# NVlabs/WarpConvNet

Hardware: AMD Instinct MI355X
Metric: M active voxels/sec fwd+bwd, SparseConv3d 64→128 k=3, 1/2/4/8 MI355X (higher is better)
Workload: dtype bf16; 1 GPU; configs[1]: one 1000000-voxel uniform (U) scene per GPU, SparseConv3d 64->128 k=3, bf16 autocast, kernel-map build + AB fwd + ABt dgrad + AtB wgrad per step; voxels_per_gpu=1000000, coord_order=generator, parallelism=dp1 (scene-sharded, grad all-reduce)

## Files before the change

warpconvnet_amd/csrc/kmap.hip:

```cpp
#include "kmap_cells.h"

namespace wcn {

constexpr int kBlockRows = 256;
constexpr int kThreads = 256;

__global__ void hash_prepare_kernel(uint4* __restrict__ slots, int64_t capacity) {
  const int64_t i = (int64_t)blockIdx.x * blockDim.x + threadIdx.x;
  if (i < capacity) slots[i] = make_uint4(0u, 0u, 0xFFFFFFFFu, 0u);
}

__global__ void hash_insert_kernel(Slot* __restrict__ slots, uint32_t capacity_mask, const int4* __restrict__ coords,
                                   int64_t n, int32_t* __restrict__ status) {
  const int64_t i = (int64_t)blockIdx.x * blockDim.x + threadIdx.x;
  if (i >= n) return;
  const int4 c = coords[i];
  if (!coord_in_range(c.x, c.y, c.z, c.w)) {
    atomicOr(status, (int)WCN_FLAG_COORD_RANGE);
    return;
  }
  const uint64_t key = pack_key(c.x, c.y, c.z, c.w);
  uint32_t s = hash_slot(key, capacity_mask);
  for (uint32_t attempts = 0; attempts <= capacity_mask; ++attempts) {
    unsigned long long* kp = reinterpret_cast<unsigned long long*>(&slots[s].key);
    const unsigned long long prev = atomicCAS(kp, 0ull, (unsigned long long)key);
    if (prev == 0ull || prev == key) {
      atomicMin(reinterpret_cast<unsigned int*>(&slots[s].value), (unsigned int)i);
      if (prev == key) atomicOr(status, (int)WCN_FLAG_DUPLICATE_COORD);
      return;
    }
    s = (s + 1) & capacity_mask;
  }
  atomicOr(status, (int)WCN_FLAG_TABLE_FULL);
}

__global__ void hash_search_kernel(const Slot* __restrict__ slots, uint32_t capacity_mask,
                                   const int4* __restrict__ queries, int64_t m, int32_t* __restrict__ results) {
  const int64_t i = (int64_t)blockIdx.x * blockDim.x + threadIdx.x;
  if (i >= m) return;
  const int4 q = queries[i];
  results[i] = slot_lookup(slots, capacity_mask, pack_key(q.x, q.y, q.z, q.w));
}

struct HashLookup {
  const Slot* slots;
  uint32_t cmask;
  __device__ __forceinline__ int operator()(int b, int x, int y, int z) const {
    return slot_lookup(slots, cmask, pack_key(b, x, y, z));
  }
};

struct CellLookup {
  const BSlot* slots;
  uint32_t cmask;
  CellTable t;
  __device__ __forceinline__ int operator()(int b, int x, int y, int z) const {
    const int xx = (x << (32 - kCoordBits)) >> (32 - kCoordBits);
    const int yy = (y << (32 - kCoordBits)) >> (32 - kCoordBits);
    const int zz = (z << (32 - kCoordBits)) >> (32 - kCoordBits);
    const int id = block_id_of(slots, cmask, make_int4(b, xx, yy, zz));
    int found = -1;
    if (id >= 0)
      found = t.cells[(int64_t)id * kCells + (((xx & (kBlk - 1)) * kBlk + (yy & (kBlk - 1))) * kBlk + (zz & (kBlk - 1)))];
    return found;
  }
};

template <int LPR, typename Lookup>
__global__ __launch_bounds__(kThreads) void kmap_probe_kernel(Lookup lookup, const int4* __restrict__ query, int64_t m,
                                                              KernelGeom g, int K, int kp, int mw, int32_t* __restrict__ nbr,
                                                              uint32_t* __restrict__ mask) {
  const int tid = threadIdx.x;
  constexpr int kRowsPerIter = 64 / LPR;
  const int lane = tid & 63;
  const int wave = tid >> 6;
  const int sub = lane % LPR;
  const int rsel = lane / LPR;
  const int64_t wave_row0 = (int64_t)blockIdx.x * kBlockRows + wave * 64;
  const int num_chunks = (kp + LPR - 1) / LPR;

  for (int kc = 0; kc < num_chunks; ++kc) {
    const int k = kc * LPR + sub;
    const bool k_real = k < K;
    const bool k_store = k < kp;
    const int l = k % g.kz;
    const int j = (k / g.kz) % g.ky;
    const int i = k / (g.kz * g.ky);
    const int ox = (i - g.cx) * g.dx, oy = (j - g.cy) * g.dy, oz = (l - g.cz) * g.dz;
#pragma unroll 4
    for (int it = 0; it < 64 / kRowsPerIter; ++it) {
      const int64_t row = wave_row0 + it * kRowsPerIter + rsel;
      int found = -1;
      if (row < m && k_real) {
        const int4 q = query[row];
        found = lookup(q.x, q.y * g.sx + ox, q.z * g.sy + oy, q.w * g.sz + oz);
      }
      if (row < m && k_store) nbr[row * kp + k] = found;
      const unsigned long long ball = __ballot(found >= 0);
      if (row < m && sub == 0) {
        const unsigned long long bits = (LPR == 64) ? ball : ((ball >> (rsel * LPR)) & ((1ull << (LPR & 63)) - 1ull));
        const int w0 = (kc * LPR) >> 5;
        if (w0 < mw) mask[row * mw + w0] = (uint32_t)bits;
        if (LPR == 64 && w0 + 1 < mw) mask[row * mw + w0 + 1] = (uint32_t)(bits >> 32);
      }
    }
  }
}

template <typename Lookup>
static int launch_probe(const Lookup& lookup, const void* table, const int32_t* query, int64_t m, const int32_t ksize[3],
                        const int32_t stride[3], const int32_t dilation[3], int32_t* nbr, uint32_t* mask, hipStream_t s) {
  if (m < 0 || !ksize || !stride || !dilation) return WCN_ERROR_INVALID_PARAMETERS;
  for (int d = 0; d < 3; ++d)
    if (ksize[d] < 1 || stride[d] < 1 || dilation[d] < 1) return WCN_ERROR_INVALID_PARAMETERS;
  const int64_t K64 = (int64_t)ksize[0] * ksize[1] * ksize[2];
  if (!valid_k(K64)) return WCN_ERROR_PROBLEM_NOT_SUPPORTED;
  if (m == 0) return WCN_SUCCESS;
  if (!table || !query || !nbr || !mask) return WCN_ERROR_INVALID_PARAMETERS;
  const int K = (int)K64, kp = wcn_kmap_row_pitch(K), mw = wcn_kmap_mask_words(K);
  const KernelGeom g = make_kernel_geom(ksize, stride, dilation);
  const dim3 grid((unsigned)ceil_div(m, kBlockRows)), block(kThreads);
#define WCN_PROBE(L) \
  hipLaunchKernelGGL((kmap_probe_kernel<L, Lookup>), grid, block, 0, s, lookup, (const int4*)query, m, g, K, kp, mw, nbr, mask)
  switch (lanes_per_row(kp)) {
    case 8: WCN_PROBE(8); break;
    case 16: WCN_PROBE(16); break;
    case 32: WCN_PROBE(32); break;
    default: WCN_PROBE(64); break;
  }
#undef WCN_PROBE
  return launch_status();
}

__global__ __launch_bounds__(256) void batch_indexed_coords_kernel(const int32_t* __restrict__ coords, int64_t n, int d,
                                                                   const int32_t* __restrict__ offsets, int num_batches,
                                                                   int32_t* __restrict__ out) {
  const int64_t i = (int64_t)blockIdx.x * blockDim.x + threadIdx.x;
  if (i >= n) return;
  const int b = last_offset_not_above(offsets, num_batches, i);
  if (d == 3) {
    const int32_t* c = coords + i * 3;
    *reinterpret_cast<int4*>(out + i * 4) = make_int4(b, c[0], c[1], c[2]);
  } else {
    out[i * (d + 1)] = b;
    for (int j = 0; j < d; ++j) out[i * (d + 1) + 1 + j] = coords[i * d + j];
  }
}

__device__ __forceinline__ uint64_t spread3(uint64_t v) {
  v &= 0x1FFFFFull;
  v = (v | (v << 32)) & 0x001F00000000FFFFull;
  v = (v | (v << 16)) & 0x001F0000FF0000FFull;
  v = (v | (v << 8)) & 0x100F00F00F00F00Full;
  v = (v | (v << 4)) & 0x10C30C30C30C30C3ull;
  v = (v | (v << 2)) & 0x1249249249249249ull;
  return v;
}

__global__ __launch_bounds__(256) void morton_code_kernel(const int32_t* __restrict__ coords, int64_t n, int d,
                                                          const int32_t* __restrict__ origin, int a0, int a1, int a2,
                                                          int64_t* __restrict__ codes) {
  const int64_t i = (int64_t)blockIdx.x * blockDim.x + threadIdx.x;
  if (i >= n) return;
  const int32_t* c = coords + i * d;
  const int sp = d - 3;
  int64_t v[3];
  const int ax[3] = {a0, a1, a2};
#pragma unroll
  for (int j = 0; j < 3; ++j) v[j] = (int64_t)c[sp + ax[j]] - (origin ? (int64_t)origin[sp + ax[j]] : 0);
  uint64_t m = spread3((uint64_t)v[0]) | (spread3((uint64_t)v[1]) << 1) | (spread3((uint64_t)v[2]) << 2);
  if (d == 4) {
    const int64_t b = (int64_t)c[0] - (origin ? (int64_t)origin[0] : 0);
    m = (m & 0x0000FFFFFFFFFFFFull) | ((uint64_t)b << 48);
  }
  codes[i] = (int64_t)m;
}

__global__ __launch_bounds__(kThreads) void kmap_transpose_kernel(const int32_t* __restrict__ nbr, int64_t m, int K,
                                                                  int kp, int tr, int32_t* __restrict__ pair_table) {
  extern __shared__ int s_tile[];
  const int64_t row0 = (int64_t)blockIdx.x * tr;
  const int pitch = kp + 1;
  for (int e = threadIdx.x; e < tr * kp; e += kThreads) {
    const int r = e / kp, k = e % kp;
    s_tile[r * pitch + k] = (row0 + r < m) ? nbr[(row0 + r) * kp + k] : -1;
  }
  __syncthreads();
  for (int e = threadIdx.x; e < tr * K; e += kThreads) {
    const int k = e / tr, r = e % tr;
    if (row0 + r < m) pair_table[(int64_t)k * m + row0 + r] = s_tile[r * pitch + k];
  }
}

__global__ void fill_i32_kernel(int32_t* __restrict__ p, int64_t n, int32_t v) {
  const int64_t i = (int64_t)blockIdx.x * blockDim.x + threadIdx.x;
  if (i < n) p[i] = v;
}

__global__ void kmap_pairs_to_table_kernel(const int32_t* __restrict__ in_maps, const int32_t* __restrict__ out_maps,
                                           const int32_t* __restrict__ offsets, int K, int kp, int mw, int64_t max_pairs,
                                           int by_in, int32_t* __restrict__ tbl, uint32_t* __restrict__ mask) {
  const int64_t p = (int64_t)blockIdx.x * blockDim.x + threadIdx.x;
  if (p >= max_pairs || p >= offsets[K]) return;
  const int k = last_offset_not_above(offsets, K, p);
  const int i = in_maps[p], o = out_maps[p];
  const int64_t row = by_in ? i : o;
  tbl[row * kp + k] = by_in ? o : i;
  atomicOr(&mask[row * mw + (k >> 5)], 1u << (k & 31));
}

}

using namespace wcn;

extern "C" {

int wcn_abi_version(void) { return 18; }

const char* wcn_status_string(int status) {
  switch (status) {
    case WCN_SUCCESS: return "Success";
    case WCN_ERROR_PROBLEM_NOT_SUPPORTED: return "Problem size not supported";
    case WCN_ERROR_KERNEL_INITIALIZATION: return "Kernel initialization failed";
    case WCN_ERROR_KERNEL_EXECUTION: return "Kernel execution failed";
    case WCN_ERROR_UNSUPPORTED_CONFIG: return "Unsupported precision/configuration";
    case WCN_ERROR_INVALID_PARAMETERS: return "Invalid parameters";
    case WCN_ERROR_MIXED_INPUT_UNSUPPORTED: return "Mixed input precision unsupported";
    default: return "Unknown error";
  }
}

static inline bool is_pow2(int64_t v) { return v > 0 && (v & (v - 1)) == 0; }

int wcn_hash_prepare(void* slots, int64_t capacity, wcn_stream_t stream) {
  if (!slots || !is_pow2(capacity) || capacity > (1ll << 31)) return WCN_ERROR_INVALID_PARAMETERS;
  hipLaunchKernelGGL(hash_prepare_kernel, dim3((unsigned)ceil_div(capacity, 256)), dim3(256), 0, (hipStream_t)stream,
                     (uint4*)slots, capacity);
  return launch_status();
}

int wcn_hash_insert(void* slots, int64_t capacity, const int32_t* coords, int64_t n, int32_t* status,
                    wcn_stream_t stream) {
  if (!slots || !is_pow2(capacity) || capacity > (1ll << 31) || n < 0 || !status) return WCN_ERROR_INVALID_PARAMETERS;
  if (n == 0) return WCN_SUCCESS;
  if (!coords) return WCN_ERROR_INVALID_PARAMETERS;
  hipLaunchKernelGGL(hash_insert_kernel, dim3((unsigned)ceil_div(n, 256)), dim3(256), 0, (hipStream_t)stream,
                     (Slot*)slots, (uint32_t)(capacity - 1), (const int4*)coords, n, status);
  return launch_status();
}

int wcn_hash_search(const void* slots, int64_t capacity, const int32_t* queries, int64_t m, int32_t* results,
                    wcn_stream_t stream) {
  if (!slots || !is_pow2(capacity) || m < 0) return WCN_ERROR_INVALID_PARAMETERS;
  if (m == 0) return WCN_SUCCESS;
  if (!queries || !results) return WCN_ERROR_INVALID_PARAMETERS;
  hipLaunchKernelGGL(hash_search_kernel, dim3((unsigned)ceil_div(m, 256)), dim3(256), 0, (hipStream_t)stream,
                     (const Slot*)slots, (uint32_t)(capacity - 1), (const int4*)queries, m, results);
  return launch_status();
}

int32_t wcn_kmap_row_pitch(int32_t num_offsets) { return (num_offsets + 7) & ~7; }
int32_t wcn_kmap_mask_words(int32_t num_offsets) { return (num_offsets + 31) / 32; }
int wcn_kmap_probe(const void* slots, int64_t capacity, const int32_t* query, int64_t m, const int32_t ksize[3],
                   const int32_t stride[3], const int32_t dilation[3], int32_t* nbr, uint32_t* mask,
                   wcn_stream_t stream) {
  if (!slots || !is_pow2(capacity)) return WCN_ERROR_INVALID_PARAMETERS;
  return launch_probe(HashLookup{(const Slot*)slots, (uint32_t)(capacity - 1)}, slots, query, m, ksize, stride, dilation, nbr,
                      mask, (hipStream_t)stream);
}

int wcn_kmap_probe_cells(const void* cells_workspace, int64_t n_in, int64_t max_blocks, const int32_t* query, int64_t m,
                         const int32_t ksize[3], const int32_t stride[3], const int32_t dilation[3], int32_t* nbr,
                         uint32_t* mask, wcn_stream_t stream) {
  if (n_in < 0 || max_blocks < 1) return WCN_ERROR_INVALID_PARAMETERS;
  const CellTable t = carve_cells(const_cast<void*>(cells_workspace), n_in, max_blocks);
  return launch_probe(CellLookup{t.slots, (uint32_t)(t.capacity - 1), t}, cells_workspace, query, m, ksize, stride, dilation,
                      nbr, mask, (hipStream_t)stream);
}

int wcn_batch_indexed_coords(const int32_t* coords, int64_t n, int32_t num_dims, const int32_t* offsets,
                             int32_t num_batches, int32_t* out, wcn_stream_t stream) {
  if (n < 0 || num_dims < 1 || num_dims > 8 || num_batches < 1) return WCN_ERROR_INVALID_PARAMETERS;
  if (n == 0) return WCN_SUCCESS;
  if (!coords || !out || (num_batches > 1 && !offsets)) return WCN_ERROR_INVALID_PARAMETERS;
  hipLaunchKernelGGL(batch_indexed_coords_kernel, dim3((unsigned)ceil_div(n, 256)), dim3(256), 0, (hipStream_t)stream, coords,
                     n, (int)num_dims, offsets, (int)num_batches, out);
  return launch_status();
}

int wcn_morton_code(const int32_t* coords, int64_t n, int32_t num_dims, const int32_t* origin, const int32_t axis[3],
                    int64_t* codes, wcn_stream_t stream) {
  if (n < 0 || (num_dims != 3 && num_dims != 4) || !axis) return WCN_ERROR_INVALID_PARAMETERS;
  int seen = 0;
  for (int j = 0; j < 3; ++j) {
    if (axis[j] < 0 || axis[j] > 2) return WCN_ERROR_INVALID_PARAMETERS;
    seen |= 1 << axis[j];
  }
  if (seen != 7) return WCN_ERROR_INVALID_PARAMETERS;
  if (n == 0) return WCN_SUCCESS;
  if (!coords || !codes) return WCN_ERROR_INVALID_PARAMETERS;
  hipLaunchKernelGGL(morton_code_kernel, dim3((unsigned)ceil_div(n, 256)), dim3(256), 0, (hipStream_t)stream, coords, n,
                     (int)num_dims, origin, (int)axis[0], (int)axis[1], (int)axis[2], codes);
  return launch_status();
}

int wcn_kmap_transpose(const int32_t* nbr, int64_t m, int32_t num_offsets, int32_t* pair_table, wcn_stream_t stream) {
  if (m < 0 || !valid_k(num_offsets)) return WCN_ERROR_INVALID_PARAMETERS;
  if (m == 0) return WCN_SUCCESS;
  if (!nbr || !pair_table) return WCN_ERROR_INVALID_PARAMETERS;
  const int kp = wcn_kmap_row_pitch(num_offsets);
  int tr = 64;
  while (tr > 1 && (size_t)tr * (kp + 1) * sizeof(int) > 64 * 1024) tr >>= 1;
  hipLaunchKernelGGL(kmap_transpose_kernel, dim3((unsigned)ceil_div(m, tr)), dim3(kThreads),
                     (size_t)tr * (kp + 1) * sizeof(int), (hipStream_t)stream, nbr, m, (int)num_offsets, kp, tr, pair_table);
  return launch_status();
}

static int pairs_to_table(const int32_t* in_maps, const int32_t* out_maps, const int32_t* offsets, int32_t K,
                          int64_t max_pairs, int64_t rows, int by_in, int32_t* tbl, uint32_t* mask, hipStream_t s) {
  if (!valid_k(K) || rows < 0 || max_pairs < 0 || !offsets) return WCN_ERROR_INVALID_PARAMETERS;
  if (rows == 0) return WCN_SUCCESS;
  if (!tbl || !mask) return WCN_ERROR_INVALID_PARAMETERS;
  const int kp = wcn_kmap_row_pitch(K), mw = wcn_kmap_mask_words(K);
  hipLaunchKernelGGL(fill_i32_kernel, dim3((unsigned)ceil_div(rows * kp, 256)), dim3(256), 0, s, tbl, rows * kp, -1);
  hipLaunchKernelGGL(fill_i32_kernel, dim3((unsigned)ceil_div(rows * mw, 256)), dim3(256), 0, s, (int32_t*)mask,
                     rows * mw, 0);
  if (max_pairs > 0) {
    if (!in_maps || !out_maps) return WCN_ERROR_INVALID_PARAMETERS;
    hipLaunchKernelGGL(kmap_pairs_to_table_kernel, dim3((unsigned)ceil_div(max_pairs, 256)), dim3(256), 0, s, in_maps,
                       out_maps, offsets, (int)K, kp, mw, max_pairs, by_in, tbl, mask);
  }
  return launch_status();
}

int wcn_kmap_reverse(const int32_t* in_maps, const int32_t* out_maps, const int32_t* offsets, int32_t num_offsets,
                     int64_t max_pairs, int64_t n_in, int32_t* rev_nbr, uint32_t* rev_mask, wcn_stream_t stream) {
  return pairs_to_table(in_maps, out_maps, offsets, num_offsets, max_pairs, n_in, 1, rev_nbr, rev_mask,
                        (hipStream_t)stream);
}

int wcn_kmap_from_csr(const int32_t* in_maps, const int32_t* out_maps, const int32_t* offsets, int32_t num_offsets,
                      int64_t max_pairs, int64_t n_out, int32_t* nbr, uint32_t* mask, wcn_stream_t stream) {
  return pairs_to_table(in_maps, out_maps, offsets, num_offsets, max_pairs, n_out, 0, nbr, mask, (hipStream_t)stream);
}

}
```

warpconvnet_amd/csrc/kmap_binned.hip:

```cpp
#include "kmap_cells.h"

namespace wcn {

constexpr int kInsertSample = 8;
constexpr int kInsertThreads = 512;
constexpr int kRowBufPitch = 66;
constexpr int kRowBufInts = (kCompactPitch + 1) * kRowBufPitch;
#ifndef WCN_NB_WPE
#define WCN_NB_WPE 3
#endif
constexpr int kNbWavesPerSimd = WCN_NB_WPE;
constexpr int kNbThreads = 256;

__device__ __forceinline__ int wrap_blk(int v) {
  const int bits = kBlkCoordBits;
  v &= (1 << bits) - 1;
  return (v ^ (1 << (bits - 1))) - (1 << (bits - 1));
}

__global__ void cell_prepare_kernel(uint4* __restrict__ slots, int64_t capacity, int32_t* __restrict__ ctr,
                                    uint32_t* __restrict__ halo, CellGeom g, int32_t* __restrict__ status) {
  const int64_t i = (int64_t)blockIdx.x * blockDim.x + threadIdx.x;
  if (i < capacity) slots[i] = make_uint4(0u, 0u, 0xFFFFFFFFu, 0u);
  if (i < 64) ctr[i] = 0;
  if (i == 0) *status = 0;
  if (i < g.halo_cells) {
    const int h3[3] = {g.hx, g.hy, g.hz};
    int t = (int)i, dir = 0;
    int sx = 0, sy = 0, sz = 0;
    for (; dir < 27; ++dir) {
      if (dir == 13) continue;
      const int dd[3] = {dir / 9 - 1, (dir / 3) % 3 - 1, dir % 3 - 1};
      sx = dd[0] ? h3[0] : kBlk; sy = dd[1] ? h3[1] : kBlk; sz = dd[2] ? h3[2] : kBlk;
      const int cells = sx * sy * sz;
      if (t < cells) break;
      t -= cells;
    }
    const int ddx = dir / 9 - 1, ddy = (dir / 3) % 3 - 1, ddz = dir % 3 - 1;
    const int tz = t % sz, ty = (t / sz) % sy, tx = t / (sz * sy);
    const int lx = ddx < 0 ? kBlk - g.hx + tx : tx;
    const int ly = ddy < 0 ? kBlk - g.hy + ty : ty;
    const int lz = ddz < 0 ? kBlk - g.hz + tz : tz;
    const int X = lx + kBlk * ddx + g.hx, Y = ly + kBlk * ddy + g.hy, Z = lz + kBlk * ddz + g.hz;
    halo[i] = ((uint32_t)dir << 27) | ((uint32_t)cell_index(lx, ly, lz) << 16) | (uint32_t)(X * g.px + Y * g.py + Z);
  }
}

__device__ __forceinline__ void store_cell(int32_t* cell, int row, bool strict) {
  if (strict) __hip_atomic_fetch_min(reinterpret_cast<uint32_t*>(cell), (uint32_t)row, __ATOMIC_RELAXED, __HIP_MEMORY_SCOPE_AGENT);
  else *cell = row;
}

template <int PHASE>
__global__ __launch_bounds__(kInsertThreads) void cell_insert_kernel(BSlot* __restrict__ slots, uint32_t cmask,
                                                          const int4* __restrict__ coords, int64_t n, CellTable t,
                                                          int32_t* __restrict__ status, int kp, int mw,
                                                          int32_t* __restrict__ nbr, uint32_t* __restrict__ mask,
                                                          int strict) {
  const bool compact = kp < 0;
  kp &= 0x7FFFFFFF;
  const int64_t tid = (int64_t)blockIdx.x * blockDim.x + threadIdx.x;
  const int64_t i = PHASE == 0 ? tid * kInsertSample : tid;
  const int lane = threadIdx.x & 63;
  bool live = i < n;
  int4 c = make_int4(0, 0, 0, 0);
  if (live) {
    c = coords[i];
    if (!coord_in_range(c.x, c.y, c.z, c.w)) {
      live = false;
      if (PHASE == 1) {
        atomicOr(status, (int)WCN_FLAG_COORD_RANGE);
        for (int k = 0; k < kp; ++k) nbr[i * kp + k] = compact ? 0 : -1;
        for (int w = 0; w < mw; ++w) mask[i * mw + w] = 0u;
      }
    }
  }
  int found = -1;
  int id = -1;
  bool created = false;
  uint64_t key = 0;
  if (live) {
    key = pack_key(c.x, c.y >> kBlkShift, c.z >> kBlkShift, c.w >> kBlkShift);
    uint32_t s = hash_slot(key, cmask);
    int idv = -1;
    for (uint32_t a = 0; a <= cmask; ++a) {
      unsigned long long* kptr = reinterpret_cast<unsigned long long*>(&slots[s].key);
      const uint4 v = *reinterpret_cast<const uint4*>(slots + s);
      unsigned long long cur = ((unsigned long long)v.y << 32) | v.x;
      if (cur == key) { found = (int)s; idv = (int)v.z; break; }
      if (cur == 0ull) {
        if (PHASE == 1) cur = __hip_atomic_load(kptr, __ATOMIC_RELAXED, __HIP_MEMORY_SCOPE_AGENT);
        if (cur == 0ull) {
          cur = atomicCAS(kptr, 0ull, (unsigned long long)key);
          if (cur == 0ull) {
            created = true;
            found = (int)s;
            break;
          }
        }
        if (cur == key) { found = (int)s; break; }
      }
      s = (s + 1) & cmask;
    }
    if (found < 0) atomicOr(status, (int)WCN_FLAG_TABLE_FULL);
    if (PHASE == 1 && idv >= 0 && !(idv & kIdLateBit)) id = idv;
  }
  __shared__ int s_made[kInsertThreads / 64 + 1];
  const int wave = threadIdx.x >> 6;
  const unsigned long long makers = __ballot(created);
  if (PHASE == 0) {
    if (lane == 0) s_made[wave] = __popcll(makers);
    __syncthreads();
    if (threadIdx.x == 0) {
      int tot = 0;
      for (int w = 0; w < kInsertThreads / 64; ++w) {
        const int c = s_made[w];
        s_made[w] = tot;
        tot += c;
      }
      s_made[kInsertThreads / 64] = tot > 0 ? atomicAdd(&t.ctr[0], tot) : 0;
    }
    __syncthreads();
  }
  if (makers != 0ull) {
    int base;
    if (PHASE == 0) {
      base = s_made[kInsertThreads / 64] + s_made[wave];
    } else {
      const int leader = __ffsll((long long)makers) - 1;
      base = 0;
      if (lane == leader) base = atomicAdd(&t.ctr[0], __popcll(makers));
      base = __shfl(base, leader);
    }
    int my_id = base + __popcll(makers & ((1ull << lane) - 1ull));
    if (!created) my_id = -1;
    if (my_id >= t.max_blocks) {
      atomicOr(status, (int)WCN_FLAG_TABLE_FULL);
      my_id = -1;
    }
    if (my_id >= 0) {
      t.blk_key[my_id] = key;
      slots[found].id = my_id | (PHASE == 1 ? kIdLateBit : 0);
    }
    unsigned long long todo = makers;
    while (todo != 0ull) {
      const int src = __ffsll((long long)todo) - 1;
      todo &= todo - 1ull;
      const int bid = __shfl(my_id, src);
      if (bid >= 0) {
        int4* gcells = reinterpret_cast<int4*>(t.cells + (int64_t)bid * kCells);
        gcells[lane] = make_int4(-1, -1, -1, -1);
        gcells[lane + 64] = make_int4(-1, -1, -1, -1);
      }
    }
  }
  if (PHASE == 0) return;
  if (live) mask[i * mw + (mw - 1)] = (id >= 0 || found < 0) ? kMaskUnwritten : kMaskDeferred;
  if (id >= 0) store_cell(t.cells + (int64_t)id * kCells + cell_of(c), (int)i, strict != 0);
}

__global__ __launch_bounds__(256) void cell_finish_kernel(const BSlot* __restrict__ slots, uint32_t cmask,
                                                          const int4* __restrict__ coords, int64_t n, CellTable t,
                                                          CellGeom g, int mw, const uint32_t* __restrict__ mask,
                                                          int strict) {
  const int64_t tid = (int64_t)blockIdx.x * blockDim.x + threadIdx.x;
  const int64_t nthreads = (int64_t)gridDim.x * blockDim.x;
  for (int64_t i = tid; i < n; i += nthreads) {
    if (mask[i * mw + (mw - 1)] != kMaskDeferred) continue;
    const int4 c = coords[i];
    const int id = block_id_of(slots, cmask, c);
    if (id < 0) continue;
    store_cell(t.cells + (int64_t)id * kCells + cell_of(c), (int)i, strict != 0);
  }
  const int lane = threadIdx.x & 63;
  int nblocks = t.ctr[0];
  if (nblocks > t.max_blocks) nblocks = (int)t.max_blocks;
  for (int64_t seq = tid >> 6; seq < nblocks; seq += nthreads >> 6) {
    const int id = (int)seq;
    int nid = -1;
    if (lane < 27) {
      const int ddx = lane / 9 - 1, ddy = (lane / 3) % 3 - 1, ddz = lane % 3 - 1;
      const bool needed = (ddx == 0 || g.hx > 0) && (ddy == 0 || g.hy > 0) && (ddz == 0 || g.hz > 0);
      if (lane == 13) nid = id;
      else if (needed) {
        const uint64_t key = t.blk_key[id];
        const int b = (int)((key >> 54) & kBatchMask);
        const int bx = wrap_blk((int)((key >> 36) & kCoordMask));
        const int by = wrap_blk((int)((key >> 18) & kCoordMask));
        const int bz = wrap_blk((int)(key & kCoordMask));
        const int s = block_find(slots, cmask, pack_key(b, wrap_blk(bx + ddx), wrap_blk(by + ddy), wrap_blk(bz + ddz)));
        if (s >= 0) {
          nid = slots[s].id;
          if (nid >= 0) nid &= ~kIdLateBit;
        }
      }
    }
    if (lane < 32) t.nbtab[(int64_t)id * 32 + lane] = nid;
  }
}

#ifdef WCN_PROF
__device__ unsigned long long g_bprof[4096 * 12];
#define BSTAMP(i) do { const unsigned long long now_ = wall_clock64(); prof_acc[i] += now_ - prof_prev; prof_prev = now_; } while (0)
#else
#define BSTAMP(i)
#endif

template <int LPR, bool FAST, bool COMPACT>
__global__ __launch_bounds__(kNbThreads) __attribute__((amdgpu_waves_per_eu(kNbWavesPerSimd))) void cell_neighbors_kernel(CellTable t, const uint32_t* __restrict__ halo,
                                                                    CellGeom g, int K, int kp, int mw,
                                                                    int32_t* __restrict__ nbr,
                                                                    uint32_t* __restrict__ mask,
                                                                    int32_t* __restrict__ status) {
  extern __shared__ int s_mem[];
  const int lane = threadIdx.x & 63, wave = threadIdx.x >> 6;
  uint32_t* s_halo = reinterpret_cast<uint32_t*>(s_mem);
  const int rounds = (g.halo_cells + 63) >> 6;
  const bool halo_regs = COMPACT && rounds <= 8;
  const int halo_pad = halo_regs ? 0 : rounds * 64;
  const int per_wave = g.cells + 4 + kCells / 2 + 8 + (COMPACT ? kRowBufInts : 0);
  int* s_grid = s_mem + halo_pad + wave * per_wave;
  unsigned short* s_own = reinterpret_cast<unsigned short*>(s_grid + g.cells + 4);
  const int null_cell = g.cells;
  for (int h = threadIdx.x; h < halo_pad; h += blockDim.x) s_halo[h] = h < g.halo_cells ? halo[h] : 0xFFFFFFFFu;
  if (lane == 0) s_grid[null_cell] = -1;
  __syncthreads();

  int nblocks = t.ctr[0];
  if (nblocks > t.max_blocks) nblocks = (int)t.max_blocks;
  const int gwave = blockIdx.x * (blockDim.x / 64) + wave;
  const int nwaves = gridDim.x * (blockDim.x / 64);
  constexpr int kVoxPerIter = 64 / LPR;
  const int sub = lane % LPR, vsel = lane / LPR;
  const int num_chunks = (kp + LPR - 1) / LPR;
  uint32_t he[8];
#pragma unroll
  for (int u = 0; u < 8; ++u) {
    const int idx = u * 64 + lane;
    uint32_t e = COMPACT && idx < g.halo_cells ? halo[idx] : 0xFFFFFFFFu;
    if (e == 0xFFFFFFFFu) e = (31u << 27) | (uint32_t)(g.cells + 1);
    he[u] = e;
  }
  auto load_head = [&](int seq, int& nb, int4& v0, int4& v1) {
    nb = -1;
    v0 = make_int4(-1, -1, -1, -1);
    v1 = v0;
    if (seq < nblocks) {
      if (lane < 27) nb = t.nbtab[(int64_t)seq * 32 + lane];
      const int4* own = reinterpret_cast<const int4*>(t.cells + (int64_t)seq * kCells) + lane * 2;
      v0 = own[0];
      v1 = own[1];
    }
  };
  int seq = gwave;
  int nb_c, nb_n;
  int4 c0, c1, n0, n1;
  load_head(seq, nb_c, c0, c1);
  load_head(seq + nwaves, nb_n, n0, n1);
  int hv[8];
  auto gather = [&](int nb, int r0) {
#pragma unroll
    for (int u = 0; u < 8; ++u) {
      hv[u] = -1;
      if (r0 + u < rounds) {
        const uint32_t e = s_halo[(r0 + u) * 64 + lane];
        const int nid = __shfl(nb, (int)((e >> 27) & 31u));
        if (e != 0xFFFFFFFFu && nid >= 0) hv[u] = t.cells[(int64_t)nid * kCells + ((e >> 16) & (kCells - 1))];
      }
    }
  };
  int nidv[8];
  auto gather8 = [&](int nb) {
#pragma unroll
    for (int u = 0; u < 8; ++u) nidv[u] = __shfl(nb, (int)(he[u] >> 27));
#pragma unroll
    for (int u = 0; u < 8; ++u)
      if (u < rounds) {
        const int safe = nidv[u] < 0 ? 0 : nidv[u];
        hv[u] = t.cells[(int64_t)safe * kCells + ((he[u] >> 16) & (kCells - 1))];
      }
  };
  auto scatter8 = [&]() {
#pragma unroll
    for (int u = 0; u < 8; ++u)
      if (u < rounds) s_grid[he[u] & 0xFFFFu] = nidv[u] >= 0 ? hv[u] : -1;
  };
  auto scatter_halo = [&](int r0) {
#pragma unroll
    for (int u = 0; u < 8; ++u)
      if (r0 + u < rounds) {
        const uint32_t e = s_halo[(r0 + u) * 64 + lane];
        if (e != 0xFFFFFFFFu) s_grid[e & 0xFFFFu] = hv[u];
      }
  };
  int* s_rows = s_grid + g.cells + 4 + kCells / 2 + 8;
  int pend_row = -1;
  auto flush_rows = [&](int row) {
    __builtin_amdgcn_fence(__ATOMIC_RELEASE, "wavefront");
    __builtin_amdgcn_wave_barrier();
    if (row >= 0) mask[row] = (uint32_t)s_rows[lane];
    const int piece = lane & 3;
    int rid[4];
    int4 v[4];
#pragma unroll
    for (int q = 0; q < 4; ++q) rid[q] = __shfl(row, (lane >> 2) + 16 * q);
#pragma unroll
    for (int q = 0; q < 4; ++q) {
      const int r = (lane >> 2) + 16 * q;
      v[q].x = s_rows[(piece * 4 + 0) * kRowBufPitch + r];
      v[q].y = s_rows[(piece * 4 + 1) * kRowBufPitch + r];
      v[q].z = s_rows[(piece * 4 + 2) * kRowBufPitch + r];
      v[q].w = s_rows[(piece * 4 + 3) * kRowBufPitch + r];
    }
#pragma unroll
    for (int q = 0; q < 4; ++q)
      if (rid[q] >= 0 && __popc((uint32_t)s_rows[(lane >> 2) + 16 * q]) >= 4 * piece) {
        if (FAST)
          *reinterpret_cast<int4*>(reinterpret_cast<char*>(nbr) + (__umul24((uint32_t)rid[q], kCompactPitch * 4u) + (uint32_t)piece * 16u)) = v[q];
        else
          *reinterpret_cast<int4*>(nbr + (int64_t)rid[q] * kCompactPitch + piece * 4) = v[q];
      }
    __builtin_amdgcn_fence(__ATOMIC_ACQUIRE, "wavefront");
    __builtin_amdgcn_wave_barrier();
  };
#ifdef WCN_PROF
  if (lane == 0 && gwave < 4096) g_bprof[gwave * 12 + 9] = wall_clock64();
#endif
  if (seq < nblocks) {
    if (halo_regs) gather8(nb_c);
    else gather(nb_c, 0);
  }
#ifdef WCN_PROF
  unsigned long long prof_prev = wall_clock64(), prof_acc[8] = {0, 0, 0, 0, 0, 0, 0, 0}, prof_blocks = 0;
  const unsigned long long prof_loop0 = prof_prev;
#endif
  for (; seq < nblocks; seq += nwaves) {
    BSTAMP(0);
#ifdef WCN_PROF
    ++prof_blocks;
#endif
    if (halo_regs) scatter8();
    else scatter_halo(0);
    for (int r0 = 8; r0 < rounds; r0 += 8) {
      gather(nb_c, r0);
      scatter_halo(r0);
    }
    BSTAMP(1);
    const int vals[8] = {c0.x, c0.y, c0.z, c0.w, c1.x, c1.y, c1.z, c1.w};
    const int cell0 = ((lane >> 3) + g.hx) * g.px + ((lane & 7) + g.hy) * g.py + g.hz;
    int mine = 0;
#pragma unroll
    for (int z = 0; z < 8; ++z) {
      s_grid[cell0 + z] = vals[z];
      mine += vals[z] >= 0;
    }
    int incl = mine;
#pragma unroll
    for (int d = 1; d < 64; d <<= 1) {
      const int up = __shfl_up(incl, d);
      if (lane >= d) incl += up;
    }
    const int own_cnt = __shfl(incl, 63);
    int at = incl - mine;
#pragma unroll
    for (int z = 0; z < 8; ++z)
      if (vals[z] >= 0) s_own[at++] = (unsigned short)((cell0 + z) * 4);
    if (lane < 2 * kVoxPerIter) s_own[own_cnt + lane] = (unsigned short)(null_cell * 4);
    BSTAMP(4);
    if (COMPACT) {
      flush_rows(pend_row);
      pend_row = -1;
    }
    BSTAMP(5);
    nb_c = nb_n; c0 = n0; c1 = n1;
    if (seq + nwaves < nblocks) {
      if (halo_regs) gather8(nb_c);
      else gather(nb_c, 0);
    }
    BSTAMP(6);
    load_head(seq + 2 * nwaves, nb_n, n0, n1);
    __builtin_amdgcn_fence(__ATOMIC_RELEASE, "wavefront");
    __builtin_amdgcn_wave_barrier();
    BSTAMP(2);
    const char* grid_bytes = reinterpret_cast<const char*>(s_grid);
    if (COMPACT) {
      int delta_lane = 0;
      if (lane < K) {
        const int l = lane % g.kz, j = (lane / g.kz) % g.ky, i = lane / (g.kz * g.ky);
        delta_lane = ((i - g.cx) * g.dx * g.px + (j - g.cy) * g.dy * g.py + (l - g.cz) * g.dz) * 4;
      }
      bool over = false;
      char* rows_bytes = reinterpret_cast<char*>(s_rows);
      const int origin4 = (g.hx * g.px + g.hy * g.py + g.hz) * 4;
      const uint32_t wp0 = (uint32_t)(kRowBufPitch + lane) * 4u, wp_max = (uint32_t)(kCompactPitch * kRowBufPitch + lane) * 4u;
      for (int e0 = 0; e0 < own_cnt; e0 += 64) {
        const bool live = e0 + lane < own_cnt;
        const int cell = live ? (int)s_own[e0 + lane] : origin4;
        const int row = live ? *reinterpret_cast<const int*>(grid_bytes + cell) : -1;
        uint32_t wp = wp0, rev = 0;
        auto answer = [&](int f) {
          *reinterpret_cast<int*>(rows_bytes + wp) = f;
          const uint32_t h = f >= 0 ? 1u : 0u;
          rev = (rev << 1) | h;
          wp = min(wp + h * (uint32_t)(kRowBufPitch * 4), wp_max);
        };
        int k = 0;
        for (; k + 4 <= K; k += 4) {
          int f[4];
#pragma unroll
          for (int u = 0; u < 4; ++u)
            f[u] = *reinterpret_cast<const int*>(grid_bytes + cell + __builtin_amdgcn_readlane(delta_lane, k + u));
#pragma unroll
          for (int u = 0; u < 4; ++u) answer(f[u]);
        }
        for (; k < K; ++k) answer(*reinterpret_cast<const int*>(grid_bytes + cell + __builtin_amdgcn_readlane(delta_lane, k)));
        const uint32_t m = __brev(rev) >> (32 - K);
        over = over || (live && __popc(m) > kCompactIds);
        s_rows[lane] = (int)m;
        if (e0 + 64 < own_cnt) flush_rows(row);
        else pend_row = row;
      }
      if (__any(over) && lane == 0) atomicOr(status, (int)WCN_FLAG_ROW_OVERFLOW);
    } else
    for (int kc = 0; kc < num_chunks; ++kc) {
      const int k = kc * LPR + sub;
      const bool k_real = k < K, k_store = k < kp;
      const int l = k % g.kz, j = (k / g.kz) % g.ky, i = k / (g.kz * g.ky);
      const int ox = (i - g.cx) * g.dx, oy = (j - g.cy) * g.dy, oz = (l - g.cz) * g.dz;
      const int delta4 = k_real ? (ox * g.px + oy * g.py + oz) * 4 : 0;
      const int w0 = (kc * LPR) >> 5;
      for (int e0 = 0; e0 < own_cnt; e0 += 2 * kVoxPerIter) {
        const int cell_a = s_own[e0 + vsel], cell_b = s_own[e0 + kVoxPerIter + vsel];
        const int row_a = *reinterpret_cast<const int*>(grid_bytes + cell_a);
        const int row_b = *reinterpret_cast<const int*>(grid_bytes + cell_b);
        int found_a = *reinterpret_cast<const int*>(grid_bytes + cell_a + delta4);
        int found_b = *reinterpret_cast<const int*>(grid_bytes + cell_b + delta4);
        if (!k_real) { found_a = -1; found_b = -1; }
        const unsigned long long ball_a = __ballot(found_a >= 0), ball_b = __ballot(found_b >= 0);
        uint32_t bits_a, bits_b, hi_a = 0, hi_b = 0;
        if (LPR == 64) {
          bits_a = (uint32_t)ball_a; hi_a = (uint32_t)(ball_a >> 32);
          bits_b = (uint32_t)ball_b; hi_b = (uint32_t)(ball_b >> 32);
        } else if (LPR == 32) {
          bits_a = vsel ? (uint32_t)(ball_a >> 32) : (uint32_t)ball_a;
          bits_b = vsel ? (uint32_t)(ball_b >> 32) : (uint32_t)ball_b;
        } else {
          bits_a = (uint32_t)(ball_a >> (vsel * LPR)) & ((1u << LPR) - 1u);
          bits_b = (uint32_t)(ball_b >> (vsel * LPR)) & ((1u << LPR) - 1u);
        }
        if (FAST) {
          char* nbr_b = reinterpret_cast<char*>(nbr);
          char* mask_b = reinterpret_cast<char*>(mask);
          const uint32_t kp4 = (uint32_t)kp * 4u, mw4 = (uint32_t)mw * 4u, k4 = (uint32_t)k * 4u, w4 = (uint32_t)w0 * 4u;
          if (row_a >= 0 && k_store) *reinterpret_cast<int*>(nbr_b + (__umul24((uint32_t)row_a, kp4) + k4)) = found_a;
          if (row_b >= 0 && k_store) *reinterpret_cast<int*>(nbr_b + (__umul24((uint32_t)row_b, kp4) + k4)) = found_b;
          if (sub == 0 && w0 < mw) {
            if (row_a >= 0) *reinterpret_cast<uint32_t*>(mask_b + (__umul24((uint32_t)row_a, mw4) + w4)) = bits_a;
            if (row_b >= 0) *reinterpret_cast<uint32_t*>(mask_b + (__umul24((uint32_t)row_b, mw4) + w4)) = bits_b;
            if (LPR == 64 && w0 + 1 < mw) {
              if (row_a >= 0) *reinterpret_cast<uint32_t*>(mask_b + (__umul24((uint32_t)row_a, mw4) + w4 + 4u)) = hi_a;
              if (row_b >= 0) *reinterpret_cast<uint32_t*>(mask_b + (__umul24((uint32_t)row_b, mw4) + w4 + 4u)) = hi_b;
            }
          }
        } else {
          if (row_a >= 0 && k_store) nbr[(int64_t)row_a * kp + k] = found_a;
          if (row_b >= 0 && k_store) nbr[(int64_t)row_b * kp + k] = found_b;
          if (sub == 0 && w0 < mw) {
            if (row_a >= 0) mask[(int64_t)row_a * mw + w0] = bits_a;
            if (row_b >= 0) mask[(int64_t)row_b * mw + w0] = bits_b;
            if (LPR == 64 && w0 + 1 < mw) {
              if (row_a >= 0) mask[(int64_t)row_a * mw + w0 + 1] = hi_a;
              if (row_b >= 0) mask[(int64_t)row_b * mw + w0 + 1] = hi_b;
            }
          }
        }
      }
    }
    BSTAMP(3);

    __builtin_amdgcn_fence(__ATOMIC_ACQUIRE, "wavefront");
    __builtin_amdgcn_wave_barrier();
  }
  if (COMPACT) flush_rows(pend_row);
#ifdef WCN_PROF
  if (lane == 0 && gwave < 4096) {
    for (int i = 0; i < 8; ++i) g_bprof[gwave * 12 + i] = prof_acc[i];
    g_bprof[gwave * 12 + 8] = prof_blocks;
    g_bprof[gwave * 12 + 10] = prof_loop0;
    g_bprof[gwave * 12 + 11] = wall_clock64();
  }
#endif
}

static void launch_cell_table(const CellTable& t, const CellGeom& g, const int4* coords, int64_t n, int kp, int mw, int32_t* nbr,
                              uint32_t* mask, int32_t* status, int strict, hipStream_t s) {
  const int64_t capacity = t.capacity;
  const uint32_t cmask = (uint32_t)(capacity - 1);
  const int64_t max_blocks = t.max_blocks;
  const int64_t prep = capacity > g.halo_cells ? capacity : g.halo_cells;
  hipLaunchKernelGGL(cell_prepare_kernel, dim3((unsigned)ceil_div(prep, 256)), dim3(256), 0, s, (uint4*)t.slots, capacity,
                     t.ctr, t.halo, g, status);
  const int64_t n_first = ceil_div(n, kInsertSample);
  hipLaunchKernelGGL(cell_insert_kernel<0>, dim3((unsigned)ceil_div(n_first, kInsertThreads)), dim3(kInsertThreads), 0, s, t.slots, cmask,
                     coords, n, t, status, kp, mw, nbr, mask, strict);
  hipLaunchKernelGGL(cell_insert_kernel<1>, dim3((unsigned)ceil_div(n, kInsertThreads)), dim3(kInsertThreads), 0, s, t.slots, cmask,
                     coords, n, t, status, kp, mw, nbr, mask, strict);
  {
    const int64_t work = n > 64 * max_blocks ? n : 64 * max_blocks;
    int64_t wgs = ceil_div(work, 256);
    if (wgs > 8192) wgs = 8192;
    hipLaunchKernelGGL(cell_finish_kernel, dim3((unsigned)wgs), dim3(256), 0, s, (const BSlot*)t.slots, cmask,
                       coords, n, t, g, mw, (const uint32_t*)mask, strict);
  }
}

}

using namespace wcn;

extern "C" {

size_t wcn_kmap_binned_workspace(int64_t n, int64_t max_blocks) {
  if (n < 0) n = 0;
  if (max_blocks < 1) max_blocks = 1;
  return carve_cells(nullptr, n, max_blocks).bytes;
}

int wcn_kmap_binned_supported(const int32_t ksize[3], const int32_t dilation[3]) {
  if (!ksize || !dilation) return 0;
  for (int d = 0; d < 3; ++d) {
    if (ksize[d] < 1 || dilation[d] < 1) return 0;
  }
  const int32_t unit[3] = {1, 1, 1};
  const KernelGeom g = make_kernel_geom(ksize, unit, dilation);
  if (kernel_halo(g.kx, g.cx, g.dx) > kMaxHalo || kernel_halo(g.ky, g.cy, g.dy) > kMaxHalo ||
      kernel_halo(g.kz, g.cz, g.dz) > kMaxHalo)
    return 0;
  const int64_t K = (int64_t)ksize[0] * ksize[1] * ksize[2];
  return (valid_k(K) && (K & 31) != 0) ? 1 : 0;
}

int wcn_kmap_compact_supported(int32_t num_offsets) {
  return (num_offsets >= 17 && num_offsets <= 31) ? 1 : 0;
}

int wcn_kmap_build_binned(const int32_t* coords, int64_t n, const int32_t ksize[3], const int32_t dilation[3],
                          int64_t max_blocks, int32_t strict, int32_t compact, void* workspace, size_t workspace_bytes,
                          int32_t* nbr, uint32_t* mask, int32_t* status, wcn_stream_t stream) {
  if (n < 0 || !status || max_blocks < 1 || max_blocks > (1ll << 29)) return WCN_ERROR_INVALID_PARAMETERS;
  if (!wcn_kmap_binned_supported(ksize, dilation)) return WCN_ERROR_PROBLEM_NOT_SUPPORTED;
  if (compact && (!ksize || !wcn_kmap_compact_supported(ksize[0] * ksize[1] * ksize[2]))) return WCN_ERROR_PROBLEM_NOT_SUPPORTED;
  if (n == 0) return WCN_SUCCESS;
  if (n >= (1ll << 31) || !coords || !nbr || !mask || !workspace ||
      workspace_bytes < wcn_kmap_binned_workspace(n, max_blocks))
    return WCN_ERROR_INVALID_PARAMETERS;
  hipStream_t s = (hipStream_t)stream;
  const CellTable t = carve_cells(workspace, n, max_blocks);
  const int K = ksize[0] * ksize[1] * ksize[2];
  const int kp = wcn_kmap_row_pitch(K), mw = wcn_kmap_mask_words(K);
  const CellGeom g = make_cell_geom(ksize, dilation);
  const int64_t capacity = t.capacity;
  const uint32_t cmask = (uint32_t)(capacity - 1);

  launch_cell_table(t, g, (const int4*)coords, n, compact ? (kCompactPitch | kCompactFlag) : kp, mw, nbr, mask, status, (int)strict, s);
  const int halo_rounds = (g.halo_cells + 63) >> 6;
  const int halo_pad = compact && halo_rounds <= 8 ? 0 : halo_rounds * 64;
  int nb_waves = kNbThreads / 64;
  auto shm_for = [&](int waves) {
    return ((size_t)halo_pad + (size_t)waves * (g.cells + 4 + kCells / 2 + 8 + (compact ? kRowBufInts : 0))) * 4;
  };
  while (nb_waves > 1 && shm_for(nb_waves) > 156 * 1024) nb_waves >>= 1;
  const size_t shm = shm_for(nb_waves);
  if (shm > 160 * 1024) return WCN_ERROR_PROBLEM_NOT_SUPPORTED;
  int per_cu = (int)((160 * 1024) / (shm + 512));
  if (per_cu > 8) per_cu = 8;
  if (compact && per_cu * nb_waves > 4 * kNbWavesPerSimd) per_cu = 4 * kNbWavesPerSimd / nb_waves;
  if (per_cu < 1) per_cu = 1;
  int64_t want = ceil_div(max_blocks < n ? max_blocks : n, nb_waves);
  if (want > 256 * per_cu) want = 256 * per_cu;
  const dim3 grid((unsigned)want), block(nb_waves * 64);
  if (shm > 64 * 1024) {
    static unsigned long long attr_done = 0ull;
    const int rc = once_per_device(attr_done, [] {
      bool ok = true;
      for (const void* f : {reinterpret_cast<const void*>(cell_neighbors_kernel<8, true, false>), reinterpret_cast<const void*>(cell_neighbors_kernel<8, false, false>),
                            reinterpret_cast<const void*>(cell_neighbors_kernel<16, true, false>), reinterpret_cast<const void*>(cell_neighbors_kernel<16, false, false>),
                            reinterpret_cast<const void*>(cell_neighbors_kernel<32, true, false>), reinterpret_cast<const void*>(cell_neighbors_kernel<32, false, false>),
                            reinterpret_cast<const void*>(cell_neighbors_kernel<32, true, true>), reinterpret_cast<const void*>(cell_neighbors_kernel<32, false, true>),
                            reinterpret_cast<const void*>(cell_neighbors_kernel<64, true, false>), reinterpret_cast<const void*>(cell_neighbors_kernel<64, false, false>)})
        ok = ok && hipFuncSetAttribute(f, hipFuncAttributeMaxDynamicSharedMemorySize, 160 * 1024) == hipSuccess;
      return ok;
    });
    if (rc != WCN_SUCCESS) return rc;
  }
  const bool fast = n < (1ll << 24) && n * kp * 4 < (1ll << 31);
#define WCN_CELL_NB(L, C)                                                                                                 \
  do {                                                                                                                    \
    if (fast)                                                                                                             \
      hipLaunchKernelGGL((cell_neighbors_kernel<L, true, C>), grid, block, shm, s, t, (const uint32_t*)t.halo, g, K, kp,  \
                         mw, nbr, mask, status);                                                                          \
    else                                                                                                                  \
      hipLaunchKernelGGL((cell_neighbors_kernel<L, false, C>), grid, block, shm, s, t, (const uint32_t*)t.halo, g, K, kp, \
                         mw, nbr, mask, status);                                                                          \
  } while (0)
  if (compact) {
    WCN_CELL_NB(32, true);
  } else {
    switch (lanes_per_row(kp)) {
      case 8: WCN_CELL_NB(8, false); break;
      case 16: WCN_CELL_NB(16, false); break;
      case 32: WCN_CELL_NB(32, false); break;
      default: WCN_CELL_NB(64, false); break;
    }
  }
#undef WCN_CELL_NB
  return launch_status();
}

int wcn_kmap_cells_build(const int32_t* coords, int64_t n, int64_t max_blocks, void* workspace, size_t workspace_bytes,
                         uint32_t* scratch, int32_t* status, wcn_stream_t stream) {
  if (n < 0 || !status || max_blocks < 1 || max_blocks > (1ll << 29)) return WCN_ERROR_INVALID_PARAMETERS;
  if (n == 0) return WCN_SUCCESS;
  if (n >= (1ll << 31) || !coords || !scratch || !workspace || workspace_bytes < wcn_kmap_binned_workspace(n, max_blocks))
    return WCN_ERROR_INVALID_PARAMETERS;
  const CellTable t = carve_cells(workspace, n, max_blocks);
  const int32_t one[3] = {1, 1, 1};
  const CellGeom g = make_cell_geom(one, one);
  launch_cell_table(t, g, (const int4*)coords, n, 0, 1, nullptr, scratch, status, 1, (hipStream_t)stream);
  return launch_status();
}

}

#ifdef WCN_PROF
extern "C" int wcn_debug_read_bprof(void* dst, size_t bytes) {
  return (int)hipMemcpyFromSymbol(dst, HIP_SYMBOL(wcn::g_bprof), bytes);
}
#endif
```

warpconvnet_amd/csrc/kmap_cells.h:

```cpp
#pragma once

#include "wcn_common.h"

namespace wcn {

constexpr int kBlkShift = 3;
constexpr int kBlk = 1 << kBlkShift;
constexpr int kCells = kBlk * kBlk * kBlk;
constexpr int kMaxHalo = 8;
constexpr int kBlkCoordBits = kCoordBits - kBlkShift;
constexpr uint32_t kMaskUnwritten = 0x80000000u;
constexpr uint32_t kMaskDeferred = 0x80000001u;

constexpr int kCompactPitch = 16;
constexpr int kCompactIds = kCompactPitch - 1;
constexpr int kCompactFlag = (int)0x80000000;

constexpr int kIdLateBit = 1 << 30;

struct __attribute__((aligned(16))) BSlot {
  uint64_t key;
  int32_t id;
  int32_t pad;
};

struct CellTable {
  BSlot* slots;
  int64_t capacity;
  int32_t* ctr;
  uint32_t* halo;
  uint64_t* blk_key;
  int32_t* nbtab;
  int32_t* cells;
  int64_t max_blocks;
  size_t bytes;
};

struct KernelGeom {
  int kx, ky, kz;
  int cx, cy, cz;
  int sx, sy, sz;
  int dx, dy, dz;
};

static inline KernelGeom make_kernel_geom(const int32_t ksize[3], const int32_t stride[3], const int32_t dilation[3]) {
  auto centre = [](int ks) { return (ks & 1) ? ks / 2 : 0; };
  return KernelGeom{ksize[0],  ksize[1],  ksize[2],  centre(ksize[0]), centre(ksize[1]), centre(ksize[2]),
                    stride[0], stride[1], stride[2], dilation[0],      dilation[1],      dilation[2]};
}

static inline int kernel_halo(int ks, int c, int d) {
  const int lo = c * d, hi = (ks - 1 - c) * d;
  return lo > hi ? lo : hi;
}

static inline int lanes_per_row(int kp) {
  int l = 8;
  while (l < kp && l < 64) l <<= 1;
  return l;
}

struct CellGeom {
  int kx, ky, kz, cx, cy, cz, dx, dy, dz;
  int hx, hy, hz;
  int px, py;
  int cells;
  int halo_cells;
};

static inline int64_t cell_capacity(int64_t max_blocks) {
  int64_t c = 1024;
  while (c < 2 * max_blocks) c <<= 1;
  return c;
}

static inline CellTable carve_cells(void* ws, int64_t n, int64_t max_blocks) {
  CellTable t;
  char* p = (char*)ws;
  size_t off = 0;
  auto take = [&](size_t bytes) { char* q = p ? p + off : nullptr; off += align256(bytes); return q; };
  (void)n;
  t.max_blocks = max_blocks;
  t.capacity = cell_capacity(max_blocks);
  t.ctr = (int32_t*)take(256);
  t.halo = (uint32_t*)take((size_t)16384 * 4);
  t.slots = (BSlot*)take((size_t)t.capacity * sizeof(BSlot));
  t.blk_key = (uint64_t*)take((size_t)max_blocks * 8);
  t.nbtab = (int32_t*)take((size_t)max_blocks * 32 * 4);
  t.cells = (int32_t*)take((size_t)max_blocks * kCells * 4);
  t.bytes = off;
  return t;
}

static inline CellGeom make_cell_geom(const int32_t ksize[3], const int32_t dilation[3]) {
  const int32_t unit[3] = {1, 1, 1};
  const KernelGeom k = make_kernel_geom(ksize, unit, dilation);
  CellGeom g;
  g.kx = k.kx; g.ky = k.ky; g.kz = k.kz;
  g.cx = k.cx; g.cy = k.cy; g.cz = k.cz;
  g.dx = k.dx; g.dy = k.dy; g.dz = k.dz;
  g.hx = kernel_halo(g.kx, g.cx, g.dx); g.hy = kernel_halo(g.ky, g.cy, g.dy); g.hz = kernel_halo(g.kz, g.cz, g.dz);
  const int gx = kBlk + 2 * g.hx, gy = kBlk + 2 * g.hy, gz = kBlk + 2 * g.hz;
  g.py = gz | 1;
  g.px = gy * g.py;
  g.cells = gx * g.px;
  g.halo_cells = gx * gy * gz - kCells;
  return g;
}

__device__ __forceinline__ int block_find(const BSlot* __restrict__ slots, uint32_t cmask, uint64_t key) {
  uint32_t s = hash_slot(key, cmask);
  for (uint32_t a = 0; a <= cmask; ++a) {
    const uint64_t k = slots[s].key;
    if (k == 0ull) return -1;
    if (k == key) return (int)s;
    s = (s + 1) & cmask;
  }
  return -1;
}

__device__ __forceinline__ int block_id_of(const BSlot* __restrict__ slots, uint32_t cmask, const int4& c) {
  const int s = block_find(slots, cmask, pack_key(c.x, c.y >> kBlkShift, c.z >> kBlkShift, c.w >> kBlkShift));
  if (s < 0) return -1;
  const int id = slots[s].id;
  return id < 0 ? -1 : (id & ~kIdLateBit);
}

__device__ __forceinline__ int cell_index(int x, int y, int z) { return (x * kBlk + y) * kBlk + z; }
__device__ __forceinline__ int cell_of(const int4& c) {
  return ((c.y & (kBlk - 1)) * kBlk + (c.z & (kBlk - 1))) * kBlk + (c.w & (kBlk - 1));
}

}
```

Measured before the change: 1086 M voxels/s.

## Reorder cells within 8^3 blocks into 2x2x4 sub-tiles

Changes the cell index layout inside each 8x8x8 block from linear x-y-z order to a tiled order of 2x2x4 sub-tiles. The halo table generation, the shared-grid scatter in the binned kernel, and the hash-lookup path are updated to match. The aim is better locality, so that spatially adjacent voxels that share neighbors fall in the same contiguous cell range, improving cache and LDS access for the neighbor probes. The cost is extra index arithmetic, and the halo enumeration becomes more complex, which adds risk of ordering bugs.

Measured after the change: 1071 M voxels/s. 1.4% lower.

```diff
diff --git a/warpconvnet_amd/csrc/kmap.hip b/warpconvnet_amd/csrc/kmap.hip
--- a/warpconvnet_amd/csrc/kmap.hip
+++ b/warpconvnet_amd/csrc/kmap.hip
@@ -60,8 +60,7 @@
     const int zz = (z << (32 - kCoordBits)) >> (32 - kCoordBits);
     const int id = block_id_of(slots, cmask, make_int4(b, xx, yy, zz));
     int found = -1;
-    if (id >= 0)
-      found = t.cells[(int64_t)id * kCells + (((xx & (kBlk - 1)) * kBlk + (yy & (kBlk - 1))) * kBlk + (zz & (kBlk - 1)))];
+    if (id >= 0) found = t.cells[(int64_t)id * kCells + cell_index(xx & (kBlk - 1), yy & (kBlk - 1), zz & (kBlk - 1))];
     return found;
   }
 };
diff --git a/warpconvnet_amd/csrc/kmap_binned.hip b/warpconvnet_amd/csrc/kmap_binned.hip
--- a/warpconvnet_amd/csrc/kmap_binned.hip
+++ b/warpconvnet_amd/csrc/kmap_binned.hip
@@ -37,10 +37,25 @@
       t -= cells;
     }
     const int ddx = dir / 9 - 1, ddy = (dir / 3) % 3 - 1, ddz = dir % 3 - 1;
-    const int tz = t % sz, ty = (t / sz) % sy, tx = t / (sz * sy);
-    const int lx = ddx < 0 ? kBlk - g.hx + tx : tx;
-    const int ly = ddy < 0 ? kBlk - g.hy + ty : ty;
-    const int lz = ddz < 0 ? kBlk - g.hz + tz : tz;
+    const int ax = ddx < 0 ? kBlk - g.hx : 0, ay = ddy < 0 ? kBlk - g.hy : 0, az = ddz < 0 ? kBlk - g.hz : 0;
+    int nx = 1, ny = 1, nz = 1, xl = ax, yl = ay, zl = az;
+    for (int T = 0; T < (kBlk >> kTileLogX); ++T) {
+      nx = box_in_tile(ax, sx, T, kTileLogX, xl);
+      if (nx > 0 && t < nx * sy * sz) break;
+      t -= max(nx, 0) * sy * sz;
+    }
+    for (int T = 0; T < (kBlk >> kTileLogY); ++T) {
+      ny = box_in_tile(ay, sy, T, kTileLogY, yl);
+      if (ny > 0 && t < nx * ny * sz) break;
+      t -= nx * max(ny, 0) * sz;
+    }
+    for (int T = 0; T < (kBlk >> kTileLogZ); ++T) {
+      nz = box_in_tile(az, sz, T, kTileLogZ, zl);
+      if (nz > 0 && t < nx * ny * nz) break;
+      t -= nx * ny * max(nz, 0);
+    }
+    ny = max(ny, 1); nz = max(nz, 1);
+    const int lx = xl + t / (nz * ny), ly = yl + (t / nz) % ny, lz = zl + t % nz;
     const int X = lx + kBlk * ddx + g.hx, Y = ly + kBlk * ddy + g.hy, Z = lz + kBlk * ddz + g.hz;
     halo[i] = ((uint32_t)dir << 27) | ((uint32_t)cell_index(lx, ly, lz) << 16) | (uint32_t)(X * g.px + Y * g.py + Z);
   }
@@ -347,11 +362,13 @@
     }
     BSTAMP(1);
     const int vals[8] = {c0.x, c0.y, c0.z, c0.w, c1.x, c1.y, c1.z, c1.w};
-    const int cell0 = ((lane >> 3) + g.hx) * g.px + ((lane & 7) + g.hy) * g.py + g.hz;
+    int ox, oy, oz;
+    cell_coords(lane * 8, ox, oy, oz);
+    const int cell0 = (ox + g.hx) * g.px + (oy + g.hy) * g.py + oz + g.hz;
     int mine = 0;
 #pragma unroll
     for (int z = 0; z < 8; ++z) {
-      s_grid[cell0 + z] = vals[z];
+      s_grid[cell0 + (z >> 2) * g.py + (z & 3)] = vals[z];
       mine += vals[z] >= 0;
     }
     int incl = mine;
@@ -364,7 +381,7 @@
     int at = incl - mine;
 #pragma unroll
     for (int z = 0; z < 8; ++z)
-      if (vals[z] >= 0) s_own[at++] = (unsigned short)((cell0 + z) * 4);
+      if (vals[z] >= 0) s_own[at++] = (unsigned short)((cell0 + (z >> 2) * g.py + (z & 3)) * 4);
     if (lane < 2 * kVoxPerIter) s_own[own_cnt + lane] = (unsigned short)(null_cell * 4);
     BSTAMP(4);
     if (COMPACT) {
diff --git a/warpconvnet_amd/csrc/kmap_cells.h b/warpconvnet_amd/csrc/kmap_cells.h
--- a/warpconvnet_amd/csrc/kmap_cells.h
+++ b/warpconvnet_amd/csrc/kmap_cells.h
@@ -126,9 +126,23 @@
   return id < 0 ? -1 : (id & ~kIdLateBit);
 }
 
-__device__ __forceinline__ int cell_index(int x, int y, int z) { return (x * kBlk + y) * kBlk + z; }
-__device__ __forceinline__ int cell_of(const int4& c) {
-  return ((c.y & (kBlk - 1)) * kBlk + (c.z & (kBlk - 1))) * kBlk + (c.w & (kBlk - 1));
+constexpr int kTileLogX = 1, kTileLogY = 1, kTileLogZ = 2;
+constexpr int kTileLog = kTileLogX + kTileLogY + kTileLogZ;
+__device__ __forceinline__ int cell_index(int x, int y, int z) {
+  const int tile = (((x >> kTileLogX) << (kBlkShift - kTileLogY)) | (y >> kTileLogY)) << (kBlkShift - kTileLogZ) | (z >> kTileLogZ);
+  const int in_tile = (((x & ((1 << kTileLogX) - 1)) << kTileLogY) | (y & ((1 << kTileLogY) - 1))) << kTileLogZ | (z & ((1 << kTileLogZ) - 1));
+  return (tile << kTileLog) | in_tile;
+}
+__device__ __forceinline__ int cell_of(const int4& c) { return cell_index(c.y & (kBlk - 1), c.z & (kBlk - 1), c.w & (kBlk - 1)); }
+__device__ __forceinline__ void cell_coords(int cell, int& x, int& y, int& z) {
+  const int tile = cell >> kTileLog;
+  z = ((tile & ((1 << (kBlkShift - kTileLogZ)) - 1)) << kTileLogZ) | (cell & ((1 << kTileLogZ) - 1));
+  y = (((tile >> (kBlkShift - kTileLogZ)) & ((1 << (kBlkShift - kTileLogY)) - 1)) << kTileLogY) | ((cell >> kTileLogZ) & ((1 << kTileLogY) - 1));
+  x = ((tile >> (2 * kBlkShift - kTileLogZ - kTileLogY)) << kTileLogX) | ((cell >> (kTileLogZ + kTileLogY)) & ((1 << kTileLogX) - 1));
+}
+__device__ __forceinline__ int box_in_tile(int a, int s, int T, int lw, int& lo) {
+  lo = max(a, T << lw);
+  return min(a + s, (T + 1) << lw) - lo;
 }
 
 }
```
